# nagadomi/nunif

Measured on NVIDIA H100. Metric: waifu2x_input_megapixels_per_sec, higher is better.
Workload: dtype f16

## Files before the change

nunif_b200/csrc/gemm_wgmma.cuh:

```cuda
#pragma once
#include "common.cuh"
#include <cuda.h>

namespace nb200 {

enum : int { ACT_NONE = 0, ACT_LRELU01 = 1, ACT_GELU = 2, ACT_RELU = 3 };
enum : int { OUT_NHWC = 0, OUT_PIXSHUF2 = 1, OUT_SPLIT = 2 };

struct GemmParams {
    int B, Ho, Wo, TH, TW, tiles_x, tiles_y;
    int N;
    int taps, cpt;
    int8_t tap_dx[16], tap_dy[16], tap_dyi[16];
    int n_tiles;
    const float* bias;
    int act;
    int out_mode, cout;
    int has_res, res_cy, res_cx;
    int res_before_act;
    int k2;
};

struct GemmMaps {
    CUtensorMap a, b;
    CUtensorMap o[4];
    union {
        CUtensorMap r[4];
        CUtensorMap a2;
    };
};

__device__ __forceinline__ uint32_t smem_u32(const void* p) { return (uint32_t)__cvta_generic_to_shared(p); }

__device__ __forceinline__ void mbar_init(uint64_t* bar, uint32_t count) {
    asm volatile("mbarrier.init.shared::cta.b64 [%0], %1;" ::"r"(smem_u32(bar)), "r"(count));
}
__device__ __forceinline__ void mbar_expect_tx(uint64_t* bar, uint32_t bytes) {
    asm volatile("mbarrier.arrive.expect_tx.shared::cta.b64 _, [%0], %1;" ::"r"(smem_u32(bar)), "r"(bytes) : "memory");
}
__device__ __forceinline__ void mbar_arrive(uint64_t* bar) {
    asm volatile("mbarrier.arrive.shared::cta.b64 _, [%0];" ::"r"(smem_u32(bar)) : "memory");
}
static __device__ __noinline__ void mbar_timeout() {
    printf("nb200: mbarrier wait timed out (block %d,%d thread %d)\n", blockIdx.x, blockIdx.y, threadIdx.x);
    __trap();
}
__device__ __forceinline__ void mbar_wait(uint64_t* bar, uint32_t parity) {
    const uint32_t addr = smem_u32(bar);
    uint32_t done = 0;
#pragma unroll 1
    for (uint32_t it = 0; it < (1u << 18); ++it) {
        asm volatile(
            "{\n\t.reg .pred p;\n\t"
            "mbarrier.try_wait.parity.shared::cta.b64 p, [%1], %2, %3;\n\t"
            "selp.u32 %0, 1, 0, p;\n\t}"
            : "=r"(done) : "r"(addr), "r"(parity), "r"(20000u) : "memory");
        if (done) return;
    }
    mbar_timeout();
}
__device__ __forceinline__ void fence_barrier_init() {
    asm volatile("fence.mbarrier_init.release.cluster;" ::: "memory");
    asm volatile("fence.proxy.async.shared::cta;" ::: "memory");
}
__device__ __forceinline__ void tma_load_5d(const CUtensorMap* map, uint64_t* bar, void* dst, int c0, int c1, int c2, int c3, int c4) {
    asm volatile(
        "cp.async.bulk.tensor.5d.shared::cluster.global.tile.mbarrier::complete_tx::bytes [%0], [%1, {%3, %4, %5, %6, %7}], [%2];"
        ::"r"(smem_u32(dst)), "l"(map), "r"(smem_u32(bar)), "r"(c0), "r"(c1), "r"(c2), "r"(c3), "r"(c4) : "memory");
}
__device__ __forceinline__ void tma_load_2d(const CUtensorMap* map, uint64_t* bar, void* dst, int c0, int c1) {
    asm volatile(
        "cp.async.bulk.tensor.2d.shared::cluster.global.tile.mbarrier::complete_tx::bytes [%0], [%1, {%3, %4}], [%2];"
        ::"r"(smem_u32(dst)), "l"(map), "r"(smem_u32(bar)), "r"(c0), "r"(c1) : "memory");
}
__device__ __forceinline__ void tma_load_4d(const CUtensorMap* map, uint64_t* bar, void* dst, int c0, int c1, int c2, int c3) {
    asm volatile(
        "cp.async.bulk.tensor.4d.shared::cluster.global.tile.mbarrier::complete_tx::bytes [%0], [%1, {%3, %4, %5, %6}], [%2];"
        ::"r"(smem_u32(dst)), "l"(map), "r"(smem_u32(bar)), "r"(c0), "r"(c1), "r"(c2), "r"(c3) : "memory");
}
__device__ __forceinline__ void tma_store_4d(const CUtensorMap* map, const void* src, int c0, int c1, int c2, int c3) {
    asm volatile("cp.async.bulk.tensor.4d.global.shared::cta.tile.bulk_group [%0, {%2, %3, %4, %5}], [%1];"
                 ::"l"(map), "r"(smem_u32(src)), "r"(c0), "r"(c1), "r"(c2), "r"(c3) : "memory");
}
__device__ __forceinline__ void tma_store_2d(const CUtensorMap* map, const void* src, int c0, int c1) {
    asm volatile("cp.async.bulk.tensor.2d.global.shared::cta.tile.bulk_group [%0, {%2, %3}], [%1];"
                 ::"l"(map), "r"(smem_u32(src)), "r"(c0), "r"(c1) : "memory");
}
__device__ __forceinline__ void tma_store_commit() { asm volatile("cp.async.bulk.commit_group;" ::: "memory"); }
__device__ __forceinline__ void tma_store_wait_read() { asm volatile("cp.async.bulk.wait_group.read 0;" ::: "memory"); }
__device__ __forceinline__ void fence_async_smem() { asm volatile("fence.proxy.async.shared::cta;" ::: "memory"); }
__device__ __forceinline__ void consumer_bar_sync() { asm volatile("bar.sync 1, 256;" ::: "memory"); }
__device__ __forceinline__ void tma_prefetch_desc(const CUtensorMap* map) {
    asm volatile("prefetch.tensormap [%0];" ::"l"(map) : "memory");
}
__device__ __forceinline__ bool elect_one() {
    uint32_t pred;
    asm volatile(
        "{\n\t.reg .pred p;\n\t"
        "elect.sync _|p, 0xffffffff;\n\t"
        "selp.u32 %0, 1, 0, p;\n\t}"
        : "=r"(pred));
    return pred != 0;
}
__device__ __forceinline__ void wgmma_fence() { asm volatile("wgmma.fence.sync.aligned;" ::: "memory"); }
__device__ __forceinline__ void wgmma_commit() { asm volatile("wgmma.commit_group.sync.aligned;" ::: "memory"); }
template <int N>
__device__ __forceinline__ void wgmma_wait() { asm volatile("wgmma.wait_group.sync.aligned %0;" ::"n"(N) : "memory"); }
template <int K>
__device__ __forceinline__ void wgmma_fence_operands(float (&d)[K]) {
#pragma unroll
    for (int j = 0; j < K; ++j) asm volatile("" : "+f"(d[j])::"memory");
}

template <int SWIZZLE_BYTES>
__device__ __forceinline__ uint64_t make_kmajor_desc(uint32_t saddr) {
    constexpr uint64_t layout = SWIZZLE_BYTES == 128 ? 1 : (SWIZZLE_BYTES == 64 ? 2 : 3);
    constexpr uint64_t sbo = (8 * SWIZZLE_BYTES) >> 4;
    return (uint64_t)((saddr & 0x3FFFF) >> 4) | (1ull << 16) | (sbo << 32) | (layout << 62);
}

template <int N>
__device__ void wgmma_f16(float (&d)[N / 2], uint64_t a, uint64_t b, uint32_t acc);
template <> __device__ __forceinline__ void wgmma_f16<16>(float (&d)[8], uint64_t a, uint64_t b, uint32_t acc) {
    asm volatile("{\n\t.reg .pred p;\n\tsetp.ne.b32 p, %10, 0;\n\t"
                 "wgmma.mma_async.sync.aligned.m64n16k16.f32.f16.f16 {%0, %1, %2, %3, %4, %5, %6, %7}, %8, %9, p, 1, 1, 0, 0;\n\t}"
                 : "+f"(d[0]), "+f"(d[1]), "+f"(d[2]), "+f"(d[3]), "+f"(d[4]), "+f"(d[5]), "+f"(d[6]), "+f"(d[7])
                 : "l"(a), "l"(b), "r"(acc));
}
template <> __device__ __forceinline__ void wgmma_f16<32>(float (&d)[16], uint64_t a, uint64_t b, uint32_t acc) {
    asm volatile("{\n\t.reg .pred p;\n\tsetp.ne.b32 p, %18, 0;\n\t"
                 "wgmma.mma_async.sync.aligned.m64n32k16.f32.f16.f16 {%0, %1, %2, %3, %4, %5, %6, %7, %8, %9, %10, %11, %12, %13, %14, %15}, %16, %17, p, 1, 1, 0, 0;\n\t}"
                 : "+f"(d[0]), "+f"(d[1]), "+f"(d[2]), "+f"(d[3]), "+f"(d[4]), "+f"(d[5]), "+f"(d[6]), "+f"(d[7]), "+f"(d[8]), "+f"(d[9]), "+f"(d[10]), "+f"(d[11]), "+f"(d[12]), "+f"(d[13]), "+f"(d[14]), "+f"(d[15])
                 : "l"(a), "l"(b), "r"(acc));
}
template <> __device__ __forceinline__ void wgmma_f16<48>(float (&d)[24], uint64_t a, uint64_t b, uint32_t acc) {
    asm volatile("{\n\t.reg .pred p;\n\tsetp.ne.b32 p, %26, 0;\n\t"
                 "wgmma.mma_async.sync.aligned.m64n48k16.f32.f16.f16 {%0, %1, %2, %3, %4, %5, %6, %7, %8, %9, %10, %11, %12, %13, %14, %15, %16, %17, %18, %19, %20, %21, %22, %23}, %24, %25, p, 1, 1, 0, 0;\n\t}"
                 : "+f"(d[0]), "+f"(d[1]), "+f"(d[2]), "+f"(d[3]), "+f"(d[4]), "+f"(d[5]), "+f"(d[6]), "+f"(d[7]), "+f"(d[8]), "+f"(d[9]), "+f"(d[10]), "+f"(d[11]), "+f"(d[12]), "+f"(d[13]), "+f"(d[14]), "+f"(d[15]), "+f"(d[16]), "+f"(d[17]), "+f"(d[18]), "+f"(d[19]), "+f"(d[20]), "+f"(d[21]), "+f"(d[22]), "+f"(d[23])
                 : "l"(a), "l"(b), "r"(acc));
}
template <> __device__ __forceinline__ void wgmma_f16<64>(float (&d)[32], uint64_t a, uint64_t b, uint32_t acc) {
    asm volatile("{\n\t.reg .pred p;\n\tsetp.ne.b32 p, %34, 0;\n\t"
                 "wgmma.mma_async.sync.aligned.m64n64k16.f32.f16.f16 {%0, %1, %2, %3, %4, %5, %6, %7, %8, %9, %10, %11, %12, %13, %14, %15, %16, %17, %18, %19, %20, %21, %22, %23, %24, %25, %26, %27, %28, %29, %30, %31}, %32, %33, p, 1, 1, 0, 0;\n\t}"
                 : "+f"(d[0]), "+f"(d[1]), "+f"(d[2]), "+f"(d[3]), "+f"(d[4]), "+f"(d[5]), "+f"(d[6]), "+f"(d[7]), "+f"(d[8]), "+f"(d[9]), "+f"(d[10]), "+f"(d[11]), "+f"(d[12]), "+f"(d[13]), "+f"(d[14]), "+f"(d[15]), "+f"(d[16]), "+f"(d[17]), "+f"(d[18]), "+f"(d[19]), "+f"(d[20]), "+f"(d[21]), "+f"(d[22]), "+f"(d[23]), "+f"(d[24]), "+f"(d[25]), "+f"(d[26]), "+f"(d[27]), "+f"(d[28]), "+f"(d[29]), "+f"(d[30]), "+f"(d[31])
                 : "l"(a), "l"(b), "r"(acc));
}
template <> __device__ __forceinline__ void wgmma_f16<96>(float (&d)[48], uint64_t a, uint64_t b, uint32_t acc) {
    asm volatile("{\n\t.reg .pred p;\n\tsetp.ne.b32 p, %50, 0;\n\t"
                 "wgmma.mma_async.sync.aligned.m64n96k16.f32.f16.f16 {%0, %1, %2, %3, %4, %5, %6, %7, %8, %9, %10, %11, %12, %13, %14, %15, %16, %17, %18, %19, %20, %21, %22, %23, %24, %25, %26, %27, %28, %29, %30, %31, %32, %33, %34, %35, %36, %37, %38, %39, %40, %41, %42, %43, %44, %45, %46, %47}, %48, %49, p, 1, 1, 0, 0;\n\t}"
                 : "+f"(d[0]), "+f"(d[1]), "+f"(d[2]), "+f"(d[3]), "+f"(d[4]), "+f"(d[5]), "+f"(d[6]), "+f"(d[7]), "+f"(d[8]), "+f"(d[9]), "+f"(d[10]), "+f"(d[11]), "+f"(d[12]), "+f"(d[13]), "+f"(d[14]), "+f"(d[15]), "+f"(d[16]), "+f"(d[17]), "+f"(d[18]), "+f"(d[19]), "+f"(d[20]), "+f"(d[21]), "+f"(d[22]), "+f"(d[23]), "+f"(d[24]), "+f"(d[25]), "+f"(d[26]), "+f"(d[27]), "+f"(d[28]), "+f"(d[29]), "+f"(d[30]), "+f"(d[31]), "+f"(d[32]), "+f"(d[33]), "+f"(d[34]), "+f"(d[35]), "+f"(d[36]), "+f"(d[37]), "+f"(d[38]), "+f"(d[39]), "+f"(d[40]), "+f"(d[41]), "+f"(d[42]), "+f"(d[43]), "+f"(d[44]), "+f"(d[45]), "+f"(d[46]), "+f"(d[47])
                 : "l"(a), "l"(b), "r"(acc));
}
template <> __device__ __forceinline__ void wgmma_f16<128>(float (&d)[64], uint64_t a, uint64_t b, uint32_t acc) {
    asm volatile("{\n\t.reg .pred p;\n\tsetp.ne.b32 p, %66, 0;\n\t"
                 "wgmma.mma_async.sync.aligned.m64n128k16.f32.f16.f16 {%0, %1, %2, %3, %4, %5, %6, %7, %8, %9, %10, %11, %12, %13, %14, %15, %16, %17, %18, %19, %20, %21, %22, %23, %24, %25, %26, %27, %28, %29, %30, %31, %32, %33, %34, %35, %36, %37, %38, %39, %40, %41, %42, %43, %44, %45, %46, %47, %48, %49, %50, %51, %52, %53, %54, %55, %56, %57, %58, %59, %60, %61, %62, %63}, %64, %65, p, 1, 1, 0, 0;\n\t}"
                 : "+f"(d[0]), "+f"(d[1]), "+f"(d[2]), "+f"(d[3]), "+f"(d[4]), "+f"(d[5]), "+f"(d[6]), "+f"(d[7]), "+f"(d[8]), "+f"(d[9]), "+f"(d[10]), "+f"(d[11]), "+f"(d[12]), "+f"(d[13]), "+f"(d[14]), "+f"(d[15]), "+f"(d[16]), "+f"(d[17]), "+f"(d[18]), "+f"(d[19]), "+f"(d[20]), "+f"(d[21]), "+f"(d[22]), "+f"(d[23]), "+f"(d[24]), "+f"(d[25]), "+f"(d[26]), "+f"(d[27]), "+f"(d[28]), "+f"(d[29]), "+f"(d[30]), "+f"(d[31]), "+f"(d[32]), "+f"(d[33]), "+f"(d[34]), "+f"(d[35]), "+f"(d[36]), "+f"(d[37]), "+f"(d[38]), "+f"(d[39]), "+f"(d[40]), "+f"(d[41]), "+f"(d[42]), "+f"(d[43]), "+f"(d[44]), "+f"(d[45]), "+f"(d[46]), "+f"(d[47]), "+f"(d[48]), "+f"(d[49]), "+f"(d[50]), "+f"(d[51]), "+f"(d[52]), "+f"(d[53]), "+f"(d[54]), "+f"(d[55]), "+f"(d[56]), "+f"(d[57]), "+f"(d[58]), "+f"(d[59]), "+f"(d[60]), "+f"(d[61]), "+f"(d[62]), "+f"(d[63])
                 : "l"(a), "l"(b), "r"(acc));
}

__device__ __forceinline__ void wgmma_f16_rs96(float (&d)[48], const uint32_t (&a)[4], uint64_t b, uint32_t acc) {
    asm volatile("{\n\t.reg .pred p;\n\tsetp.ne.b32 p, %53, 0;\n\t"
                 "wgmma.mma_async.sync.aligned.m64n96k16.f32.f16.f16 {%0, %1, %2, %3, %4, %5, %6, %7, %8, %9, %10, %11, %12, %13, %14, %15, %16, %17, %18, %19, %20, %21, %22, %23, %24, %25, %26, %27, %28, %29, %30, %31, %32, %33, %34, %35, %36, %37, %38, %39, %40, %41, %42, %43, %44, %45, %46, %47}, {%48, %49, %50, %51}, %52, p, 1, 1, 0;\n\t}"
                 : "+f"(d[0]), "+f"(d[1]), "+f"(d[2]), "+f"(d[3]), "+f"(d[4]), "+f"(d[5]), "+f"(d[6]), "+f"(d[7]), "+f"(d[8]), "+f"(d[9]), "+f"(d[10]), "+f"(d[11]), "+f"(d[12]), "+f"(d[13]), "+f"(d[14]), "+f"(d[15]), "+f"(d[16]), "+f"(d[17]), "+f"(d[18]), "+f"(d[19]), "+f"(d[20]), "+f"(d[21]), "+f"(d[22]), "+f"(d[23]), "+f"(d[24]), "+f"(d[25]), "+f"(d[26]), "+f"(d[27]), "+f"(d[28]), "+f"(d[29]), "+f"(d[30]), "+f"(d[31]), "+f"(d[32]), "+f"(d[33]), "+f"(d[34]), "+f"(d[35]), "+f"(d[36]), "+f"(d[37]), "+f"(d[38]), "+f"(d[39]), "+f"(d[40]), "+f"(d[41]), "+f"(d[42]), "+f"(d[43]), "+f"(d[44]), "+f"(d[45]), "+f"(d[46]), "+f"(d[47])
                 : "r"(a[0]), "r"(a[1]), "r"(a[2]), "r"(a[3]), "l"(b), "r"(acc));
}

__device__ __forceinline__ float gelu_erf(float x) {
    const float a = fabsf(x);
    float q = fmaf(a, 4.88118734e-04f, -7.19881030e-03f);
    q = fmaf(q, a, 5.21468017e-02f);
    q = fmaf(q, a, 4.59595724e-01f);
    q = fmaf(q, a, 1.15100057e+00f);
    float e;
    asm("ex2.approx.ftz.f32 %0, %1;" : "=f"(e) : "f"(fmaf(-q, a, -1.0f)));
    return fmaxf(x, 0.f) - a * e;
}

template <int K>
__device__ __forceinline__ void apply_act(float (&v)[K], int act) {
    switch (act) {
        case ACT_LRELU01:
#pragma unroll
            for (int j = 0; j < K; ++j) v[j] = v[j] > 0.f ? v[j] : 0.1f * v[j];
            break;
        case ACT_GELU:
#pragma unroll
            for (int j = 0; j < K; ++j) v[j] = gelu_erf(v[j]);
            break;
        case ACT_RELU:
#pragma unroll
            for (int j = 0; j < K; ++j) v[j] = fmaxf(v[j], 0.f);
            break;
        default: break;
    }
}

constexpr int GEMM_CONSUMER_THREADS = 256;
constexpr int GEMM_THREADS = GEMM_CONSUMER_THREADS + 32;

template <int BLOCK_N, int BK>
struct GemmCfg {
    static_assert(BLOCK_N % 16 == 0 && BLOCK_N <= 128, "BLOCK_N: 16..128 (the fp32 accumulators live in registers)");
    static constexpr int SWIZZLE = BK * 2;
    static constexpr int A_BYTES = 128 * BK * 2;
    static constexpr int B_BYTES = BLOCK_N * BK * 2;
    static constexpr int STAGE_BYTES = A_BYTES + ((B_BYTES + 1023) / 1024) * 1024;
    static constexpr int STAGES = (98304 / STAGE_BYTES) < 2 ? 2 : ((98304 / STAGE_BYTES) > 6 ? 6 : (98304 / STAGE_BYTES));
    static constexpr int CW = (BLOCK_N % 64 == 0) ? 64 : ((BLOCK_N % 32 == 0) ? 32 : 16);
    static constexpr int NCH = BLOCK_N / CW;
    static constexpr int CH_BYTES = 128 * CW * 2;
    static_assert(NCH * CH_BYTES <= STAGES * STAGE_BYTES, "epilogue staging must fit in the (drained) pipeline stages");
    static constexpr int SMEM_BYTES = STAGES * STAGE_BYTES + 1024  + 256 ;
// ... 157 lines not shown
```

nunif_b200/csrc/swin_attention_mma.cu:

```cuda
#include "common.cuh"
#include "gemm_wgmma.cuh"
#include "swin_kernels.h"
#include "tmap.h"
#include <map>
#include <mutex>

namespace nb200 {

extern int g_tune[16];

namespace {
constexpr int WS = 6, WTOK = 36, WPAD = 48, HEADS = 6;

__device__ __forceinline__ void mma16816(float (&c)[4], const uint32_t (&a)[4], uint32_t b0, uint32_t b1) {
    asm volatile(
        "mma.sync.aligned.m16n8k16.row.col.f32.f16.f16.f32 {%0,%1,%2,%3}, {%4,%5,%6,%7}, {%8,%9}, {%0,%1,%2,%3};"
        : "+f"(c[0]), "+f"(c[1]), "+f"(c[2]), "+f"(c[3])
        : "r"(a[0]), "r"(a[1]), "r"(a[2]), "r"(a[3]), "r"(b0), "r"(b1));
}
__device__ __forceinline__ void ldmatrix_x2_trans(uint32_t& r0, uint32_t& r1, const void* smem_row) {
    const uint32_t addr = (uint32_t)__cvta_generic_to_shared(smem_row);
    asm volatile("ldmatrix.sync.aligned.m8n8.x2.trans.shared.b16 {%0,%1}, [%2];" : "=r"(r0), "=r"(r1) : "r"(addr));
}
__device__ __forceinline__ uint32_t pack_half2(float a, float b) {
// ... 187 lines not shown
    __syncthreads();

    const int head = tid >> 5, lane = tid & 31, g = lane >> 2, t4 = lane & 3;
    const int hc = head * D;
    const float scale = ((D == 16) ? 0.25f : 0.17677669529663687f) * 1.4426950408889634f;
    const bool boundary = shift > 0 && (wy == gridDim.x / nww - 1 || wx == nww - 1);
    const float4* bf = bias_frag + (size_t)head * (3 * 6 * 32) + lane;
    AttnCtx<D> cx;
    cx.sq = sq; cx.sreg = sreg; cx.bf = bf; cx.hc = hc; cx.g = g; cx.t4 = t4; cx.scale = scale; cx.boundary = boundary;
#pragma unroll
    for (int nt = 0; nt < NKT; ++nt) cx.kbase[nt] = sk + min(nt * 8 + g, WTOK - 1) * LD + hc + 2 * t4;
    cx.vbase[0] = sv + (lane & 15) * LD + hc;
    cx.vbase[1] = sv + (16 + (lane & 15)) * LD + hc;
    cx.vbase[2] = sv + min(32 + (lane & 7), WTOK - 1) * LD + hc;
#pragma unroll 1
    for (int mt = 0; mt < 2; ++mt) attn_mtile<D, LD, false>(cx, mt);
    attn_mtile<D, LD, true>(cx, 2);
    __syncthreads();
    for (int t = rg; t < WTOK; t += RG)
        *reinterpret_cast<uint4*>(out + (size_t)stok[t] * C + vv * 8) = *reinterpret_cast<const uint4*>(sq + t * LD + vv * 8);
}

__global__ void build_bias_frag_kernel(const float* __restrict__ table, float4* __restrict__ frag) {
    const int i = blockIdx.x * blockDim.x + threadIdx.x;
    if (i >= HEADS * 3 * 6 * 32) return;
    const int lane = i & 31, nt = (i >> 5) % 6, mt = (i / (32 * 6)) % 3, head = i / (32 * 6 * 3);
    const int g = lane >> 2, t4 = lane & 3;
    float v[4];
#pragma unroll
    for (int r = 0; r < 4; ++r) {
        const int row = mt * 16 + g + 8 * (r >> 1), col = nt * 8 + 2 * t4 + (r & 1);
        if (col >= WTOK) v[r] = -1e30f;
        else if (row >= WTOK) v[r] = 0.f;
        else {
            const int qy = row / WS, qx = row % WS, ky = col / WS, kx = col % WS;
            v[r] = 1.4426950408889634f * table[((qy - ky + WS - 1) * (2 * WS - 1) + (qx - kx + WS - 1)) * HEADS + head];
        }
    }
    frag[i] = make_float4(v[0], v[1], v[2], v[3]);
}

int build_bias_frag(cudaStream_t st, const float* table, float* frag) {
    build_bias_frag_kernel<<<(HEADS * 3 * 6 * 32 + 255) / 256, 256, 0, st>>>(table, reinterpret_cast<float4*>(frag));
    NB_LAUNCHED();
    return 0;
}

template <int D>
static size_t attn_smem_bytes() {
    constexpr int C = D * HEADS, LD = C + 8;
    return (size_t)3 * WTOK * LD * 2 + (WTOK + WPAD) * 4 + 16;
}

static int set_attn_attrs(const void* func, size_t smem, int carveout) {
    static std::mutex mu;
    static std::map<std::pair<int, const void*>, int> done;
    int dev = 0;
    NB_CUDA(cudaGetDevice(&dev));
    std::lock_guard<std::mutex> lk(mu);
    int& have = done[{dev, func}];
    if (have != carveout) {
        NB_CUDA(cudaFuncSetAttribute(func, cudaFuncAttributeMaxDynamicSharedMemorySize, (int)smem));
        NB_CUDA(cudaFuncSetAttribute(func, cudaFuncAttributePreferredSharedMemoryCarveout, carveout));
        have = carveout;
    }
    return 0;
}

int window_attention(cudaStream_t st, const __half* qkv, const float* bias_frag_f, __half* out, int B, int H, int W, int C,
                     int shift, size_t plane) {
    const float4* bias_table = reinterpret_cast<const float4*>(bias_frag_f);
    NB_CHECK(H % WS == 0 && W % WS == 0, "feature map must be a multiple of the 6x6 window");
    NB_CHECK(C == 96 || C == 192, "window attention supports C=96 (d=16) and C=192 (d=32)");
    if (WS >= H) shift = 0;
    dim3 grid((H / WS) * (W / WS), B);
    ProfScope ps(st, PC_ATTN, (double)B * H * W * C * 4 * 2, (double)B * H * W * C * 3 * 2, (double)B * H * W * C * 2);
    if (C == 96) {
        const int want = g_tune[6] > 0 ? g_tune[6] : 72;
        if (set_attn_attrs((const void*)window_attention_mma_kernel<16>, attn_smem_bytes<16>(), want)) return 1;
        window_attention_mma_kernel<16><<<grid, 192, attn_smem_bytes<16>(), st>>>(qkv, bias_table, out, H, W, shift, plane);
    } else {
        const int want = g_tune[6] > 0 ? g_tune[6] : 86;
        if (set_attn_attrs((const void*)window_attention_mma_kernel<32>, attn_smem_bytes<32>(), want)) return 1;
        window_attention_mma_kernel<32><<<grid, 192, attn_smem_bytes<32>(), st>>>(qkv, bias_table, out, H, W, shift, plane);
    }
    NB_LAUNCHED();
    return 0;
}


constexpr int FA_ROWS = 128, FA_WIN = 3, FA_THREADS = GEMM_CONSUMER_THREADS + 32, FA_SLOT = 96 * 64, FA_STAGES = 4;
constexpr int FA_LD = 32 + 8;
constexpr int FA_CHUNK_BYTES = FA_WIN * 3 * WTOK * FA_LD * 2;

template <int C>
struct FaCfg {
    static constexpr int X_BYTES = FA_ROWS * C * 2;
    static constexpr int SMEM = X_BYTES + FA_STAGES * FA_SLOT + FA_CHUNK_BYTES + FA_WIN * (WTOK + WPAD) * 4 + 2 * FA_STAGES * 8 + 1024;
};

template <int C>
__global__ void __launch_bounds__(FA_THREADS, 2) swin_attn_fused_kernel(const __grid_constant__ CUtensorMap wmap,
                                                                        const __half* __restrict__ x, const float* __restrict__ bqkv,
                                                                        const float4* __restrict__ bias_frag, __half* __restrict__ out,
                                                                        int H, int W, int shift, int nwin) {
    using Cfg = FaCfg<C>;
    constexpr int D = C / HEADS, KB = C / 32, NCH = C / 32, HPC = 32 / D;
    extern __shared__ uint8_t smem_dyn[];
    uint8_t* smem = reinterpret_cast<uint8_t*>((reinterpret_cast<uintptr_t>(smem_dyn) + 1023) & ~(uintptr_t)1023);
    uint8_t* sx = smem;
    uint8_t* ring = smem + Cfg::X_BYTES;
    __half* sqkv = reinterpret_cast<__half*>(ring + FA_STAGES * FA_SLOT);
    int* stok = reinterpret_cast<int*>(reinterpret_cast<uint8_t*>(sqkv) + FA_CHUNK_BYTES);
    int* sreg = stok + FA_WIN * WTOK;
    uint64_t* full = reinterpret_cast<uint64_t*>(sreg + FA_WIN * WPAD);
    uint64_t* empty = full + FA_STAGES;
    const int tid = threadIdx.x, warp = tid >> 5;
    const int nww = W / WS, nwy = H / WS;
    if (tid < FA_WIN * WPAD) {
        const int w = tid / WPAD, t = tid % WPAD, gw = blockIdx.x * FA_WIN + w;
        int reg = -1;
        if (t < WTOK) {
            int tok = -1;
            if (gw < nwin) {
                const int b = gw / (nww * nwy), r = gw % (nww * nwy), wy = r / nww, wx = r % nww;
                const int ry = wy * WS + t / WS, rx = wx * WS + t % WS;
                const int y = (ry + shift) % H, xx = (rx + shift) % W;
                tok = (b * H + y) * W + xx;
                int hr = 0, wr = 0;
                if (shift > 0) {
                    hr = ry < H - WS ? 0 : (ry < H - shift ? 1 : 2);
                    wr = rx < W - WS ? 0 : (rx < W - shift ? 1 : 2);
                }
                reg = hr * 3 + wr;
            }
            stok[w * WTOK + t] = tok;
        }
        sreg[w * WPAD + t] = reg;
    }
    if (tid == GEMM_CONSUMER_THREADS) {
        tma_prefetch_desc(&wmap);
        for (int s = 0; s < FA_STAGES; ++s) {
            mbar_init(&full[s], 1);
            mbar_init(&empty[s], 2);
        }
        fence_barrier_init();
    }
    __syncthreads();
    if (tid == 0) NB_PDL_TRIGGER();

    if (warp == GEMM_CONSUMER_THREADS / 32) {
        if (elect_one()) {
            for (int i = 0; i < NCH * KB; ++i) {
                const int s = i % FA_STAGES, c = i / KB;
                mbar_wait(&empty[s], ((i / FA_STAGES) & 1) ^ 1);
                mbar_expect_tx(&full[s], FA_SLOT);
#pragma unroll
                for (int m = 0; m < 3; ++m)
                    tma_load_2d(&wmap, &full[s], ring + s * FA_SLOT + m * 32 * 64, (i % KB) * 32, m * C + 32 * c);
            }
        }
        return;
    }

    for (int i = tid; i < FA_ROWS * (C / 8); i += GEMM_CONSUMER_THREADS) {
        const int r = i / (C / 8), u = i % (C / 8);
        uint8_t* dst = sx + (u >> 2) * (FA_ROWS * 64) + stage_off<32>(r, u & 3);
        const int tok = r < FA_WIN * WTOK ? stok[r] : -1;
        if (tok >= 0) cp_async16(dst, x + (size_t)tok * C + u * 8);
        else *reinterpret_cast<uint4*>(dst) = make_uint4(0u, 0u, 0u, 0u);
    }
    asm volatile("cp.async.commit_group;" ::: "memory");
    asm volatile("cp.async.wait_group 0;" ::: "memory");
    fence_async_smem();
    consumer_bar_sync();

    const int wg = tid >> 7, t = tid & 127;
    const int row0 = wg * 64 + (t >> 5) * 16 + ((t & 31) >> 2);
    const int cq = 2 * (t & 3);
    const uint32_t a_base = smem_u32(sx) + wg * 64 * 64;
    const int lane = tid & 31, g = lane >> 2, t4 = lane & 3;
    const float scale = ((D == 16) ? 0.25f : 0.17677669529663687f) * 1.4426950408889634f;
#pragma unroll 1
    for (int c = 0; c < NCH; ++c) {
        float acc[48];
#pragma unroll
        for (int j = 0; j < 48; ++j) acc[j] = 0.f;
#pragma unroll 1
        for (int kb = 0; kb < KB; ++kb) {
            const int it = c * KB + kb, s = it % FA_STAGES;
            mbar_wait(&full[s], (it / FA_STAGES) & 1);
            const uint32_t a = a_base + kb * (FA_ROWS * 64), bb = smem_u32(ring + s * FA_SLOT);
            wgmma_fence();
            wgmma_f16<96>(acc, make_kmajor_desc<64>(a), make_kmajor_desc<64>(bb), 1u);
            wgmma_f16<96>(acc, make_kmajor_desc<64>(a + 32), make_kmajor_desc<64>(bb + 32), 1u);
            wgmma_commit();
            wgmma_wait<1>();
            if (kb > 0 && t == 0) mbar_arrive(&empty[(it - 1) % FA_STAGES]);
        }
        wgmma_wait<0>();
        if (t == 0) mbar_arrive(&empty[(c * KB + KB - 1) % FA_STAGES]);
        wgmma_fence_operands(acc);
        consumer_bar_sync();
#pragma unroll
        for (int j = 0; j < 12; ++j) {
            const int m = j >> 2, col = 8 * (j & 3) + cq;
            const float2 bq = __ldg(reinterpret_cast<const float2*>(bqkv + m * C + 32 * c + col));
#pragma unroll
            for (int i = 0; i < 2; ++i) {
                const int r = row0 + 8 * i;
                if (r < FA_WIN * WTOK) {
                    const int w = r / WTOK, tk = r - w * WTOK;
                    *reinterpret_cast<__half2*>(sqkv + ((w * 3 + m) * WTOK + tk) * FA_LD + col) =
                        __floats2half2_rn(acc[4 * j + 2 * i] + bq.x, acc[4 * j + 2 * i + 1] + bq.y);
                }
            }
        }
        consumer_bar_sync();

#pragma unroll 1
        for (int item = warp; item < 3 * FA_WIN * HPC; item += GEMM_CONSUMER_THREADS / 32) {
            const int mt = item / (FA_WIN * HPC), pr = item - mt * (FA_WIN * HPC), w = pr / HPC, hh = pr - w * HPC;
            const int gw = blockIdx.x * FA_WIN + w;
            if (gw >= nwin) continue;
            const int r = gw % (nww * nwy), wy = r / nww, wx = r % nww, head = c * HPC + hh;
            __half* sq = sqkv + w * 3 * WTOK * FA_LD;
            __half* sk = sq + WTOK * FA_LD;
            __half* sv = sk + WTOK * FA_LD;
            AttnCtx<D> cx;
            cx.sq = sq; cx.sreg = sreg + w * WPAD; cx.bf = bias_frag + (size_t)head * (3 * 6 * 32) + lane;
            cx.hc = hh * D; cx.g = g; cx.t4 = t4; cx.scale = scale;
            cx.boundary = shift > 0 && (wy == nwy - 1 || wx == nww - 1);
#pragma unroll
            for (int nt = 0; nt < NKT; ++nt) cx.kbase[nt] = sk + min(nt * 8 + g, WTOK - 1) * FA_LD + cx.hc + 2 * t4;
            cx.vbase[0] = sv + (lane & 15) * FA_LD + cx.hc;
            cx.vbase[1] = sv + (16 + (lane & 15)) * FA_LD + cx.hc;
            cx.vbase[2] = sv + min(32 + (lane & 7), WTOK - 1) * FA_LD + cx.hc;
            if (mt < 2) attn_mtile<D, FA_LD, false>(cx, mt);
            else attn_mtile<D, FA_LD, true>(cx, 2);
            __syncwarp();
            const int nrow = mt < 2 ? 16 : WTOK - 32;
            for (int e = lane; e < nrow * (D / 8); e += 32) {
                const int tk = 16 * mt + e / (D / 8), u = e % (D / 8);
                *reinterpret_cast<uint4*>(out + (size_t)stok[w * WTOK + tk] * C + head * D + u * 8) =
                    *reinterpret_cast<const uint4*>(sq + tk * FA_LD + cx.hc + u * 8);
            }
        }
    }
}

int swin_attn_fused(cudaStream_t st, const __half* x, const __half* wqkv, const float* bqkv, const float* bias_frag_f, __half* att,
                    int B, int H, int W, int C, int shift) {
    NB_CHECK(x && wqkv && bqkv && bias_frag_f && att, "null pointer");
    NB_CHECK(H % WS == 0 && W % WS == 0, "feature map must be a multiple of the 6x6 window");
    NB_CHECK(C == 96 || C == 192, "fused window attention supports C=96 (d=16) and C=192 (d=32)");
    if (WS >= H) shift = 0;
    const long long nwin = (long long)B * (H / WS) * (W / WS);
    NB_CHECK(nwin > 0 && nwin < (1LL << 31), "window count out of range");
    CUtensorMap wmap;
    const cuuint64_t dims[2] = {(cuuint64_t)C, (cuuint64_t)(3 * C)};
    const cuuint64_t strides[1] = {(cuuint64_t)C * 2};
    const cuuint32_t box[2] = {32, 32};
    if (encode(&wmap, wqkv, 2, dims, strides, box, 64)) return 1;
    const double T = (double)B * H * W;
    ProfScope ps(st, PC_FUSED_ATTN, T * 3.0 * C * C * 2 + T * C * 36 * 4, T * C * 2, T * C * 2);
    const unsigned grid = (unsigned)((nwin + FA_WIN - 1) / FA_WIN);
    const float4* bf = reinterpret_cast<const float4*>(bias_frag_f);
    if (C == 96) {
        if (ensure_dyn_smem((const void*)swin_attn_fused_kernel<96>, FaCfg<96>::SMEM)) return 1;
        swin_attn_fused_kernel<96><<<grid, FA_THREADS, FaCfg<96>::SMEM, st>>>(wmap, x, bqkv, bf, att, H, W, shift, (int)nwin);
    } else {
        if (ensure_dyn_smem((const void*)swin_attn_fused_kernel<192>, FaCfg<192>::SMEM)) return 1;
        swin_attn_fused_kernel<192><<<grid, FA_THREADS, FaCfg<192>::SMEM, st>>>(wmap, x, bqkv, bf, att, H, W, shift, (int)nwin);
    }
    NB_LAUNCHED();
    return 0;
}

}
```

nunif_b200/csrc/swin_block.cu:

```cuda
#include "gemm_wgmma.cuh"
#include "swin_kernels.h"
#include "tmap.h"

namespace nb200 {

constexpr int FM_ROWS = 128, FM_STAGES = 5, FM_THREADS = GEMM_CONSUMER_THREADS + 128;
constexpr int FM_PRODUCER_REGS = 40, FM_CONSUMER_REGS = 232;

template <int C>
struct FmCfg {
    static constexpr int KB = C / 32;
    static constexpr int TILE = FM_ROWS * C * 2;
    static constexpr int STAGE = 128 * C;
    static constexpr int SMEM = 2 * TILE + FM_STAGES * STAGE + (2 * FM_STAGES + KB + 1) * 8 + 1024;
};

struct FmMaps {
    CUtensorMap x, att, wp, w1, w2, y, wy;
};

template <int K>
__device__ __forceinline__ float (&half96(float (&acc)[K], int h))[48] { return *reinterpret_cast<float(*)[48]>(&acc[48 * h]); }

__device__ __forceinline__ void fm_wait(uint64_t* bar, uint32_t parity) {
    const uint32_t addr = smem_u32(bar);
    uint32_t done = 0;
#pragma unroll 1
    for (uint32_t it = 0; it < (1u << 18) && !done; ++it)
        asm volatile(
            "{\n\t.reg .pred p;\n\t"
            "mbarrier.try_wait.parity.shared::cta.b64 p, [%1], %2, %3;\n\t"
            "selp.u32 %0, 1, 0, p;\n\t}"
            : "=r"(done) : "r"(addr), "r"(parity), "r"(20000u) : "memory");
    if (!done) __trap();
}

__device__ __forceinline__ void wgmma_wait_n(int n) {
    if (n == 0) wgmma_wait<0>();
    else wgmma_wait<1>();
}

template <int C, bool PROJ, int CS>
__global__ void __launch_bounds__(FM_THREADS, 1) swin_mlp_fused_kernel(const __grid_constant__ FmMaps maps, const float* __restrict__ bp,
                                                                     const float* __restrict__ b1, const float* __restrict__ b2,
                                                                     const float* __restrict__ by) {
    using Cfg = FmCfg<C>;
    static_assert(CS % 16 == 0 && 2 * C * CS <= Cfg::STAGE && CS * 256 <= Cfg::TILE, "Wy must fit a ring stage, y the att tile");
    constexpr int KB = Cfg::KB, NP = (KB + 1) / 2, NH = 2 * C / 64, NHALF = C / 96;
    extern __shared__ uint8_t smem_dyn[];
    uint8_t* smem = reinterpret_cast<uint8_t*>((reinterpret_cast<uintptr_t>(smem_dyn) + 1023) & ~(uintptr_t)1023);
    uint8_t* sx = smem;
    uint8_t* satt = smem + Cfg::TILE;
    uint8_t* ring = smem + 2 * Cfg::TILE;
    uint64_t* full = reinterpret_cast<uint64_t*>(ring + FM_STAGES * Cfg::STAGE);
    uint64_t* empty = full + FM_STAGES;
    uint64_t* abar = empty + FM_STAGES;
    uint64_t* xbar = abar + KB;
    const int tid = threadIdx.x, warp = tid >> 5;
    const int row_base = blockIdx.x * FM_ROWS;
    if (tid == GEMM_CONSUMER_THREADS) {
        tma_prefetch_desc(&maps.x);
        tma_prefetch_desc(&maps.w1);
        tma_prefetch_desc(&maps.w2);
        if (CS) tma_prefetch_desc(&maps.wy);
        if (PROJ) {
            tma_prefetch_desc(&maps.att);
            tma_prefetch_desc(&maps.wp);
        }
        for (int s = 0; s < FM_STAGES; ++s) {
            mbar_init(&full[s], 1);
            mbar_init(&empty[s], 2);
        }
        for (int kb = 0; kb < KB; ++kb) mbar_init(&abar[kb], 1);
        mbar_init(xbar, 1);
        fence_barrier_init();
    }
    __syncthreads();

    if (warp >= GEMM_CONSUMER_THREADS / 32) {
        asm volatile("setmaxnreg.dec.sync.aligned.u32 %0;" ::"n"(FM_PRODUCER_REGS));
        if (warp == GEMM_CONSUMER_THREADS / 32 && elect_one()) {
            bool acts = false;
            auto load_acts = [&]() {
                asm volatile("griddepcontrol.wait;" ::: "memory");
                if (PROJ)
                    for (int kb = 0; kb < KB; ++kb) {
                        mbar_expect_tx(&abar[kb], FM_ROWS * 64);
                        tma_load_2d(&maps.att, &abar[kb], satt + kb * (FM_ROWS * 64), kb * 32, row_base);
                    }
                mbar_expect_tx(xbar, Cfg::TILE);
                for (int kb = 0; kb < KB; ++kb) tma_load_2d(&maps.x, xbar, sx + kb * (FM_ROWS * 64), kb * 32, row_base);
                acts = true;
            };
            int it = 0;
            auto push = [&](const CUtensorMap* m, int k0, int n0, int rows, int nbox) {
                if (it == FM_STAGES) load_acts();
                const int s = it % FM_STAGES;
                fm_wait(&empty[s], ((it / FM_STAGES) & 1) ^ 1);
                mbar_expect_tx(&full[s], nbox * rows * 64);
                for (int b = 0; b < nbox; ++b) tma_load_2d(m, &full[s], ring + s * Cfg::STAGE + b * rows * 64, k0 + 32 * b, n0);
                ++it;
            };
            if (PROJ)
                for (int j = 0; j < NP; ++j) push(&maps.wp, 64 * j, 0, C, min(2, KB - 2 * j));
            push(&maps.w1, 0, 0, 64, KB);
            for (int hc = 0; hc < NH; ++hc) {
                if (hc + 1 < NH) push(&maps.w1, 0, (hc + 1) * 64, 64, KB);
                push(&maps.w2, hc * 64, 0, C, 2);
            }
            if (CS) push(&maps.wy, 0, 0, CS, KB);
            if (!acts) load_acts();
        }
        return;
    }

    asm volatile("setmaxnreg.inc.sync.aligned.u32 %0;" ::"n"(FM_CONSUMER_REGS));
    const int wg = tid >> 7, t = tid & 127;
    const int row0 = wg * 64 + (t >> 5) * 16 + ((t & 31) >> 2);
    const int cq = 2 * (t & 3);
    const uint32_t x_base = smem_u32(sx) + wg * 64 * 64, att_base = smem_u32(satt) + wg * 64 * 64;
    int it = 0, pending = 0;
    auto take = [&]() -> uint32_t {
        const int s = it % FM_STAGES;
        fm_wait(&full[s], (it / FM_STAGES) & 1);
        return smem_u32(ring + s * Cfg::STAGE);
    };
    auto commit = [&]() {
        wgmma_commit();
        ++it;
        ++pending;
    };
    auto retire = [&](int n) {
        wgmma_wait_n(n);
#pragma unroll
        for (int k = 0; k < FM_STAGES; ++k)
            if (k < pending - n && t == 0) mbar_arrive(&empty[(it - pending + k) % FM_STAGES]);
        pending = min(pending, n);
    };

    if (PROJ) {
        float acc[C / 2];
#pragma unroll
        for (int j = 0; j < C / 2; ++j) acc[j] = 0.f;
        wgmma_fence_operands(acc);
#pragma unroll
        for (int j = 0; j < NP; ++j) {
            const uint32_t bb = take();
#pragma unroll
            for (int kb = 2 * j; kb < 2 * j + 2 && kb < KB; ++kb) fm_wait(&abar[kb], 0);
            wgmma_fence();
#pragma unroll
            for (int kb = 2 * j; kb < 2 * j + 2 && kb < KB; ++kb) {
                const uint32_t a = att_base + kb * (FM_ROWS * 64), b = bb + (kb - 2 * j) * (C * 64);
#pragma unroll
                for (int s = 0; s < 2; ++s)
#pragma unroll
                    for (int h = 0; h < NHALF; ++h)
                        wgmma_f16<96>(half96(acc, h), make_kmajor_desc<64>(a + 32 * s), make_kmajor_desc<64>(b + h * 96 * 64 + 32 * s), 1u);
            }
            commit();
            retire(1);
        }
        retire(0);
        wgmma_fence_operands(acc);
        fm_wait(xbar, 0);
#pragma unroll
        for (int j = 0; j < C / 8; ++j) {
            const int col = 8 * j + cq;
            const float2 bq = __ldg(reinterpret_cast<const float2*>(bp + col));
#pragma unroll
            for (int i = 0; i < 2; ++i) {
                __half2* p = reinterpret_cast<__half2*>(sx + sw64_off<FM_ROWS>(row0 + 8 * i, col));
                const float2 xv = __half22float2(*p);
                *p = __floats2half2_rn(xv.x + (acc[4 * j + 2 * i] + bq.x), xv.y + (acc[4 * j + 2 * i + 1] + bq.y));
            }
        }
        fence_async_smem();
        asm volatile("bar.sync %0, 128;" ::"r"(2 + wg) : "memory");
    } else {
        fm_wait(xbar, 0);
    }

    float oacc[C / 2];
#pragma unroll
    for (int j = 0; j < C / 2; ++j) oacc[j] = 0.f;
    wgmma_fence_operands(oacc);
    float hacc[2][32];
    uint32_t af[4][4];
    auto fc1 = [&](float (&h)[32]) {
#pragma unroll
        for (int j = 0; j < 32; ++j) h[j] = 0.f;
        wgmma_fence_operands(h);
        const uint32_t bb = take();
        wgmma_fence();
#pragma unroll
        for (int kb = 0; kb < KB; ++kb) {
            const uint32_t a = x_base + kb * (FM_ROWS * 64), b = bb + kb * (64 * 64);
            wgmma_f16<64>(h, make_kmajor_desc<64>(a), make_kmajor_desc<64>(b), 1u);
            wgmma_f16<64>(h, make_kmajor_desc<64>(a + 32), make_kmajor_desc<64>(b + 32), 1u);
        }
        commit();
    };
    fc1(hacc[0]);
#pragma unroll
    for (int hc = 0; hc < NH; ++hc) {
        const int buf = hc & 1;
        if (hc + 1 < NH) fc1(hacc[buf ^ 1]);
        retire(hc + 1 < NH ? 1 : 0);
        wgmma_fence_operands(hacc[buf]);
#pragma unroll
        for (int kk = 0; kk < 4; ++kk)
#pragma unroll
            for (int q = 0; q < 4; ++q) {
                const int j = 2 * kk + (q >> 1), i = q & 1;
                const float2 bq = __ldg(reinterpret_cast<const float2*>(b1 + 64 * hc + 8 * j + cq));
                const __half2 h = __floats2half2_rn(gelu_erf(hacc[buf][4 * j + 2 * i] + bq.x), gelu_erf(hacc[buf][4 * j + 2 * i + 1] + bq.y));
                af[kk][q] = *reinterpret_cast<const uint32_t*>(&h);
            }
        const uint32_t bb = take();
        wgmma_fence();
#pragma unroll
        for (int kb = 0; kb < 2; ++kb)
#pragma unroll
            for (int s = 0; s < 2; ++s)
#pragma unroll
                for (int h = 0; h < NHALF; ++h)
                    wgmma_f16_rs96(half96(oacc, h), af[2 * kb + s], make_kmajor_desc<64>(bb + kb * (C * 64) + h * 96 * 64 + 32 * s), 1u);
        commit();
    }
    retire(0);
    wgmma_fence_operands(oacc);
#pragma unroll
    for (int j = 0; j < C / 8; ++j) {
        const int col = 8 * j + cq;
        const float2 bq = __ldg(reinterpret_cast<const float2*>(b2 + col));
#pragma unroll
        for (int i = 0; i < 2; ++i) {
            __half2* p = reinterpret_cast<__half2*>(sx + sw64_off<FM_ROWS>(row0 + 8 * i, col));
            const float2 xv = __half22float2(*p);
            *p = __floats2half2_rn(xv.x + (oacc[4 * j + 2 * i] + bq.x), xv.y + (oacc[4 * j + 2 * i + 1] + bq.y));
        }
    }
    fence_async_smem();
    if constexpr (CS > 0) {
        asm volatile("bar.sync %0, 128;" ::"r"(2 + wg) : "memory");
        float yacc[CS / 2];
#pragma unroll
        for (int j = 0; j < CS / 2; ++j) yacc[j] = 0.f;
        wgmma_fence_operands(yacc);
        const uint32_t bb = take();
        wgmma_fence();
#pragma unroll
        for (int kb = 0; kb < KB; ++kb) {
            const uint32_t a = x_base + kb * (FM_ROWS * 64), b = bb + kb * (CS * 64);
            wgmma_f16<CS>(yacc, make_kmajor_desc<64>(a), make_kmajor_desc<64>(b), 1u);
            wgmma_f16<CS>(yacc, make_kmajor_desc<64>(a + 32), make_kmajor_desc<64>(b + 32), 1u);
        }
        commit();
        retire(0);
        wgmma_fence_operands(yacc);
#pragma unroll
        for (int j = 0; j < CS / 8; ++j) {
            const int col = 8 * j + cq;
            const float2 bq = __ldg(reinterpret_cast<const float2*>(by + col));
#pragma unroll
            for (int i = 0; i < 2; ++i) {
                __half2* p = reinterpret_cast<__half2*>(satt + (col >> 4) * (FM_ROWS * 32) + stage_off<16>(row0 + 8 * i, (col & 15) >> 3) +
                                                        (col & 7) * 2);
                *p = __floats2half2_rn(yacc[4 * j + 2 * i] + bq.x, yacc[4 * j + 2 * i + 1] + bq.y);
            }
        }
        fence_async_smem();
    }
    consumer_bar_sync();
    if (tid == 0) {
        if constexpr (CS > 0)
            for (int c = 0; c < CS / 16; ++c) tma_store_2d(&maps.y, satt + c * (FM_ROWS * 32), 16 * c, row_base);
        else
            for (int kb = 0; kb < KB; ++kb) tma_store_2d(&maps.x, sx + kb * (FM_ROWS * 64), kb * 32, row_base);
        tma_store_commit();
        tma_store_wait_read();
    }
}

static int map2d(CUtensorMap* m, const void* base, int cols, long long rows, int box_rows) {
    const cuuint64_t dims[2] = {(cuuint64_t)cols, (cuuint64_t)rows};
    const cuuint64_t strides[1] = {(cuuint64_t)cols * 2};
    const cuuint32_t box[2] = {32, (cuuint32_t)box_rows};
    return encode(m, base, 2, dims, strides, box, 64);
}

template <int C, bool PROJ, int CS = 0>
static int launch_mlp(cudaStream_t st, unsigned grid, const FmMaps& maps, const float* bp, const float* b1, const float* b2,
                      const float* by = nullptr) {
    if (ensure_dyn_smem((const void*)swin_mlp_fused_kernel<C, PROJ, CS>, FmCfg<C>::SMEM)) return 1;
    cudaLaunchConfig_t cfg = {};
    cfg.gridDim = dim3(grid); cfg.blockDim = dim3(FM_THREADS); cfg.dynamicSmemBytes = FmCfg<C>::SMEM;
    cfg.stream = st;
    cudaLaunchAttribute at[1];
    at[0].id = cudaLaunchAttributeProgrammaticStreamSerialization;
    at[0].val.programmaticStreamSerializationAllowed = 1;
    cfg.attrs = at; cfg.numAttrs = 1;
    NB_CUDA(cudaLaunchKernelEx(&cfg, swin_mlp_fused_kernel<C, PROJ, CS>, maps, bp, b1, b2, by));
    NB_LAUNCHED();
    return 0;
}

int swin_mlp_fused(cudaStream_t st, __half* x, const __half* att, long long T, int C, const __half* wp, const float* bp,
                   const __half* w1, const float* b1, const __half* w2, const float* b2, __half* y, int cs, const __half* wy,
                   const float* by) {
    NB_CHECK(x && w1 && b1 && w2 && b2 && (!att || (wp && bp)) && (!y || (att && wy && by)), "null pointer");
    NB_CHECK(C == 96 || C == 192, "C must be 96 or 192");
    NB_CHECK(!y || (C == 192 && cs == 48) || (C == 96 && cs == 16), "y: cs must be 48 at C = 192 and 16 at C = 96");
    NB_CHECK(T > 0 && T < (1LL << 31), "token count out of range");
    FmMaps maps;
    memset(&maps, 0, sizeof(maps));
    if (map2d(&maps.x, x, C, T, FM_ROWS)) return 1;
    if (att && (map2d(&maps.att, att, C, T, FM_ROWS) || map2d(&maps.wp, wp, C, C, C))) return 1;
    if (map2d(&maps.w1, w1, C, 2 * C, 64) || map2d(&maps.w2, w2, 2 * C, C, C)) return 1;
    if (y) {
        if (map2d(&maps.wy, wy, C, cs, cs)) return 1;
        const cuuint64_t dims[2] = {(cuuint64_t)cs, (cuuint64_t)T};
        const cuuint64_t strides[1] = {(cuuint64_t)cs * 2};
        const cuuint32_t box[2] = {16, FM_ROWS};
        if (encode(&maps.y, y, 2, dims, strides, box, 32)) return 1;
    }
    const double Td = (double)T;
    ProfScope ps(st, PC_FUSED_MLP, Td * C * 2 * (C * ((att ? 1 : 0) + 4) + (y ? cs : 0)), Td * C * 2 * (att ? 2 : 1),
                 Td * (y ? cs : C) * 2);
    const unsigned grid = (unsigned)((T + FM_ROWS - 1) / FM_ROWS);
    if (y) return C == 96 ? launch_mlp<96, true, 16>(st, grid, maps, bp, b1, b2, by) : launch_mlp<192, true, 48>(st, grid, maps, bp, b1, b2, by);
    if (C == 96) return att ? launch_mlp<96, true>(st, grid, maps, bp, b1, b2) : launch_mlp<96, false>(st, grid, maps, bp, b1, b2);
    return att ? launch_mlp<192, true>(st, grid, maps, bp, b1, b2) : launch_mlp<192, false>(st, grid, maps, bp, b1, b2);
// ... 24 lines not shown
```

Before: 72.48.

## Enable programmatic dependent launch between fused attention and Swin MLP kernels

The fused attention kernel is now launched with programmatic stream serialization. It waits on griddepcontrol only before it reads activations, and the producer warp waits only after its first weight stages are issued, so weight prefetch overlaps the tail of the previous kernel. The Swin MLP kernel now also triggers the dependent launch early. The shared mbarrier wait is replaced by a lighter trap-only version (no printf), and the local fm_wait is folded into it, which cuts register and code overhead in the wait loops. The risk is correctness: if the PDL waits are placed wrong, a kernel could read activations before the previous kernel has finished writing them.

```diff
diff --git a/nunif_b200/csrc/gemm_wgmma.cuh b/nunif_b200/csrc/gemm_wgmma.cuh
--- a/nunif_b200/csrc/gemm_wgmma.cuh
+++ b/nunif_b200/csrc/gemm_wgmma.cuh
@@ -41,23 +41,17 @@
 __device__ __forceinline__ void mbar_arrive(uint64_t* bar) {
     asm volatile("mbarrier.arrive.shared::cta.b64 _, [%0];" ::"r"(smem_u32(bar)) : "memory");
 }
-static __device__ __noinline__ void mbar_timeout() {
-    printf("nb200: mbarrier wait timed out (block %d,%d thread %d)\n", blockIdx.x, blockIdx.y, threadIdx.x);
-    __trap();
-}
 __device__ __forceinline__ void mbar_wait(uint64_t* bar, uint32_t parity) {
     const uint32_t addr = smem_u32(bar);
     uint32_t done = 0;
 #pragma unroll 1
-    for (uint32_t it = 0; it < (1u << 18); ++it) {
+    for (uint32_t it = 0; it < (1u << 18) && !done; ++it)
         asm volatile(
             "{\n\t.reg .pred p;\n\t"
             "mbarrier.try_wait.parity.shared::cta.b64 p, [%1], %2, %3;\n\t"
             "selp.u32 %0, 1, 0, p;\n\t}"
             : "=r"(done) : "r"(addr), "r"(parity), "r"(20000u) : "memory");
-        if (done) return;
-    }
-    mbar_timeout();
+    if (!done) __trap();
 }
 __device__ __forceinline__ void fence_barrier_init() {
     asm volatile("fence.mbarrier_init.release.cluster;" ::: "memory");
diff --git a/nunif_b200/csrc/swin_attention_mma.cu b/nunif_b200/csrc/swin_attention_mma.cu
--- a/nunif_b200/csrc/swin_attention_mma.cu
+++ b/nunif_b200/csrc/swin_attention_mma.cu
@@ -363,6 +363,7 @@
     if (warp == GEMM_CONSUMER_THREADS / 32) {
         if (elect_one()) {
             for (int i = 0; i < NCH * KB; ++i) {
+                if (i == FA_STAGES) asm volatile("griddepcontrol.wait;" ::: "memory");
                 const int s = i % FA_STAGES, c = i / KB;
                 mbar_wait(&empty[s], ((i / FA_STAGES) & 1) ^ 1);
                 mbar_expect_tx(&full[s], FA_SLOT);
@@ -374,6 +375,7 @@
         return;
     }
 
+    asm volatile("griddepcontrol.wait;" ::: "memory");
     for (int i = tid; i < FA_ROWS * (C / 8); i += GEMM_CONSUMER_THREADS) {
         const int r = i / (C / 8), u = i % (C / 8);
         uint8_t* dst = sx + (u >> 2) * (FA_ROWS * 64) + stage_off<32>(r, u & 3);
@@ -458,6 +460,22 @@
             }
         }
     }
+}
+
+template <int C>
+static int launch_attn(cudaStream_t st, unsigned grid, const CUtensorMap& wmap, const __half* x, const float* bqkv,
+                       const float4* bf, __half* att, int H, int W, int shift, int nwin) {
+    if (ensure_dyn_smem((const void*)swin_attn_fused_kernel<C>, FaCfg<C>::SMEM)) return 1;
+    cudaLaunchConfig_t cfg = {};
+    cfg.gridDim = dim3(grid); cfg.blockDim = dim3(FA_THREADS); cfg.dynamicSmemBytes = FaCfg<C>::SMEM;
+    cfg.stream = st;
+    cudaLaunchAttribute at[1];
+    at[0].id = cudaLaunchAttributeProgrammaticStreamSerialization;
+    at[0].val.programmaticStreamSerializationAllowed = 1;
+    cfg.attrs = at; cfg.numAttrs = 1;
+    NB_CUDA(cudaLaunchKernelEx(&cfg, swin_attn_fused_kernel<C>, wmap, x, bqkv, bf, att, H, W, shift, nwin));
+    NB_LAUNCHED();
+    return 0;
 }
 
 int swin_attn_fused(cudaStream_t st, const __half* x, const __half* wqkv, const float* bqkv, const float* bias_frag_f, __half* att,
@@ -477,15 +495,8 @@
     ProfScope ps(st, PC_FUSED_ATTN, T * 3.0 * C * C * 2 + T * C * 36 * 4, T * C * 2, T * C * 2);
     const unsigned grid = (unsigned)((nwin + FA_WIN - 1) / FA_WIN);
     const float4* bf = reinterpret_cast<const float4*>(bias_frag_f);
-    if (C == 96) {
-        if (ensure_dyn_smem((const void*)swin_attn_fused_kernel<96>, FaCfg<96>::SMEM)) return 1;
-        swin_attn_fused_kernel<96><<<grid, FA_THREADS, FaCfg<96>::SMEM, st>>>(wmap, x, bqkv, bf, att, H, W, shift, (int)nwin);
-    } else {
-        if (ensure_dyn_smem((const void*)swin_attn_fused_kernel<192>, FaCfg<192>::SMEM)) return 1;
-        swin_attn_fused_kernel<192><<<grid, FA_THREADS, FaCfg<192>::SMEM, st>>>(wmap, x, bqkv, bf, att, H, W, shift, (int)nwin);
-    }
-    NB_LAUNCHED();
-    return 0;
-}
-
-}
+    return C == 96 ? launch_attn<96>(st, grid, wmap, x, bqkv, bf, att, H, W, shift, (int)nwin)
+                   : launch_attn<192>(st, grid, wmap, x, bqkv, bf, att, H, W, shift, (int)nwin);
+}
+
+}
diff --git a/nunif_b200/csrc/swin_block.cu b/nunif_b200/csrc/swin_block.cu
--- a/nunif_b200/csrc/swin_block.cu
+++ b/nunif_b200/csrc/swin_block.cu
@@ -21,19 +21,6 @@
 
 template <int K>
 __device__ __forceinline__ float (&half96(float (&acc)[K], int h))[48] { return *reinterpret_cast<float(*)[48]>(&acc[48 * h]); }
-
-__device__ __forceinline__ void fm_wait(uint64_t* bar, uint32_t parity) {
-    const uint32_t addr = smem_u32(bar);
-    uint32_t done = 0;
-#pragma unroll 1
-    for (uint32_t it = 0; it < (1u << 18) && !done; ++it)
-        asm volatile(
-            "{\n\t.reg .pred p;\n\t"
-            "mbarrier.try_wait.parity.shared::cta.b64 p, [%1], %2, %3;\n\t"
-            "selp.u32 %0, 1, 0, p;\n\t}"
-            : "=r"(done) : "r"(addr), "r"(parity), "r"(20000u) : "memory");
-    if (!done) __trap();
-}
 
 __device__ __forceinline__ void wgmma_wait_n(int n) {
     if (n == 0) wgmma_wait<0>();
@@ -76,6 +63,7 @@
         fence_barrier_init();
     }
     __syncthreads();
+    if (tid == 0) NB_PDL_TRIGGER();
 
     if (warp >= GEMM_CONSUMER_THREADS / 32) {
         asm volatile("setmaxnreg.dec.sync.aligned.u32 %0;" ::"n"(FM_PRODUCER_REGS));
@@ -96,7 +84,7 @@
             auto push = [&](const CUtensorMap* m, int k0, int n0, int rows, int nbox) {
                 if (it == FM_STAGES) load_acts();
                 const int s = it % FM_STAGES;
-                fm_wait(&empty[s], ((it / FM_STAGES) & 1) ^ 1);
+                mbar_wait(&empty[s], ((it / FM_STAGES) & 1) ^ 1);
                 mbar_expect_tx(&full[s], nbox * rows * 64);
                 for (int b = 0; b < nbox; ++b) tma_load_2d(m, &full[s], ring + s * Cfg::STAGE + b * rows * 64, k0 + 32 * b, n0);
                 ++it;
@@ -122,7 +110,7 @@
     int it = 0, pending = 0;
     auto take = [&]() -> uint32_t {
         const int s = it % FM_STAGES;
-        fm_wait(&full[s], (it / FM_STAGES) & 1);
+        mbar_wait(&full[s], (it / FM_STAGES) & 1);
         return smem_u32(ring + s * Cfg::STAGE);
     };
     auto commit = [&]() {
@@ -147,7 +135,7 @@
         for (int j = 0; j < NP; ++j) {
             const uint32_t bb = take();
 #pragma unroll
-            for (int kb = 2 * j; kb < 2 * j + 2 && kb < KB; ++kb) fm_wait(&abar[kb], 0);
+            for (int kb = 2 * j; kb < 2 * j + 2 && kb < KB; ++kb) mbar_wait(&abar[kb], 0);
             wgmma_fence();
 #pragma unroll
             for (int kb = 2 * j; kb < 2 * j + 2 && kb < KB; ++kb) {
@@ -163,7 +151,7 @@
         }
         retire(0);
         wgmma_fence_operands(acc);
-        fm_wait(xbar, 0);
+        mbar_wait(xbar, 0);
 #pragma unroll
         for (int j = 0; j < C / 8; ++j) {
             const int col = 8 * j + cq;
@@ -178,7 +166,7 @@
         fence_async_smem();
         asm volatile("bar.sync %0, 128;" ::"r"(2 + wg) : "memory");
     } else {
-        fm_wait(xbar, 0);
+        mbar_wait(xbar, 0);
     }
 
     float oacc[C / 2];
```

Result: no change. 72.27 (median of 6 runs) (-0.3%).
